# arpan-dhatt/wgpu-n-body

Measured on AMD Instinct MI355X. Metric: body-pair interactions/sec, 64k-body all-pairs, higher is better.
Workload: dtype f32; 1 GPU; 65536-body naive all-pairs step (BASELINE configs[1]), uniform_init seed 2, g=1e-6 e=1e-4 dt=0.016; bodies=65536, parallelism=body-range shard x1, lib=nbody_hip 0.2.0 gfx950 src:823fa9bfdf5b, kernel_variant=auto

## Files before the change

wgpu_n_body_amd/csrc/nb_common.hpp:

```cpp
#pragma once

#include <hip/hip_runtime.h>

#include <cstdarg>
#include <cstddef>
#include <cstdint>
#include <cstdio>
#include <string>

#include "nbody.h"

namespace nb {

void set_error(const char *fmt, ...) __attribute__((format(printf, 1, 2)));

#define NB_HIP_TRY(expr)                                                                       \
    do {                                                                                       \
        hipError_t nb_e_ = (expr);                                                             \
        if (nb_e_ != hipSuccess) {                                                             \
            ::nb::set_error("%s failed: %s (%s:%d)", #expr, hipGetErrorString(nb_e_), __FILE__, \
                            __LINE__);                                                         \
            return NB_ERR_HIP;                                                                 \
        }                                                                                      \
    } while (0)

constexpr uint32_t kWave = 64;
constexpr uint32_t kIB = 2;
constexpr uint32_t kITile = kWave * kIB;
constexpr uint32_t kJTile = 64;
constexpr uint32_t kPadTo = 256;

constexpr int kMaxPeers = 15;
struct PeerDst {
    float4 *p[kMaxPeers];
    uint32_t n;
};

struct PeerWords {
    uint32_t *p[kMaxPeers];
    uint32_t n;
};
hipError_t launch_peer_check_store(const PeerWords &dst, uint32_t slot, uint32_t value, hipStream_t stream);
hipError_t launch_peer_check_read(const uint32_t *words, uint32_t world, uint32_t me, uint32_t tag, uint32_t *bad,
                                  hipStream_t stream);

struct NaiveLaunch {
    const float4 *posm_src;
    float4 *posm_dst;
    float4 *vel;
    float4 *acc;
    uint32_t n;
    uint32_t n_pad;
    uint32_t lo, hi;
    float g, e, dt;
    int variant;
    int jsplit;
    int mass_runs;
    float4 *partial;
    uint32_t partial_stride;
    uint32_t partial_slices;
    int phase;
    PeerDst peers;
};
enum { kPhaseAll = 0, kPhaseLocal = 1, kPhaseRemote = 2 };
struct NaivePlan {
    int variant;
    uint32_t blocks;
    uint32_t jsplit;
    uint32_t js_local, js_remote;
    uint32_t n_tiles, lo_tile, local_tiles;
    bool two_phase;
};
NaivePlan plan_naive(uint32_t n, uint32_t lo, uint32_t hi, int variant, int jsplit, bool two_phase);
hipError_t launch_naive_step(const NaiveLaunch &a, hipStream_t stream);
int naive_variant_count();
const char *naive_variant_name(int v);

hipError_t launch_aos_to_soa(const nb_particle *aos, float4 *posm, float4 *vel, float4 *acc,
                             uint32_t n, uint32_t lo, uint32_t hi, hipStream_t stream);
hipError_t launch_soa_to_aos(const float4 *posm, const float4 *vel, const float4 *acc,
                             nb_particle *aos, uint32_t n, uint32_t lo, uint32_t hi,
                             hipStream_t stream);

}
```

wgpu_n_body_amd/csrc/nb_naive.hip:

```cpp
#include "nb_common.hpp"

#include <type_traits>

namespace nb {
namespace {

typedef float v2f __attribute__((ext_vector_type(2)));
typedef float v4f __attribute__((ext_vector_type(4)));

enum JSource { kLds = 0, kSmem = 1 };

struct TileWindow {
    uint32_t base, count, skip_at, skip_len;
    __device__ __forceinline__ uint32_t tile(uint32_t v) const {
        return base + v + (v >= skip_at ? skip_len : 0u);
    }
};

__device__ __forceinline__ float kick(float v, float a, float dt) {
#pragma clang fp contract(off)
    return v + (a * dt) / 2.0f;
}
__device__ __forceinline__ float drift(float x, float v, float dt) {
#pragma clang fp contract(off)
    return x + v * dt;
}

template <bool MASKED, bool UNIFORM>
__device__ __forceinline__ void pair(float xj, float yj, float zj, float mj, float xi, float yi,
                                     float zi, float e, bool valid, float &ax, float &ay,
                                     float &az) {
    const float dx = xj - xi, dy = yj - yi, dz = zj - zi;
    const float r2 = __builtin_fmaf(dz, dz, __builtin_fmaf(dy, dy, dx * dx));
    const float r = __builtin_amdgcn_sqrtf(r2);
    const float den = __builtin_fmaf(e, r, r2 * r2);
    float w = __builtin_amdgcn_rcpf(den);
    if (!UNIFORM) w *= mj;
    if (MASKED) w = valid ? w : 0.0f;
    ax = __builtin_fmaf(w, dx, ax);
    ay = __builtin_fmaf(w, dy, ay);
    az = __builtin_fmaf(w, dz, az);
}

template <bool MASKED, bool UNIFORM>
__device__ __forceinline__ void pair2(float xj, float yj, float zj, float mj, v2f xi, v2f yi,
                                      v2f zi, float e, bool valid0, bool valid1, v2f &ax,
                                      v2f &ay, v2f &az) {
    const v2f dx = v2f{xj, xj} - xi, dy = v2f{yj, yj} - yi, dz = v2f{zj, zj} - zi;
    const v2f r2 = __builtin_elementwise_fma(dz, dz, __builtin_elementwise_fma(dy, dy, dx * dx));
    v2f r;
    r.x = __builtin_amdgcn_sqrtf(r2.x);
    r.y = __builtin_amdgcn_sqrtf(r2.y);
    const v2f den = __builtin_elementwise_fma(v2f{e, e}, r, r2 * r2);
    v2f rc;
    rc.x = __builtin_amdgcn_rcpf(den.x);
    rc.y = __builtin_amdgcn_rcpf(den.y);
    v2f w = UNIFORM ? rc : v2f{mj, mj} * rc;
    if (MASKED) {
        w.x = valid0 ? w.x : 0.0f;
        w.y = valid1 ? w.y : 0.0f;
    }
    ax = __builtin_elementwise_fma(w, dx, ax);
    ay = __builtin_elementwise_fma(w, dy, ay);
    az = __builtin_elementwise_fma(w, dz, az);
}

template <int IB, int SRC, bool PACKED, bool MASKED, bool UNIFORM, int UNROLL, typename Ptr,
          typename T>
__device__ __forceinline__ void tile_body(Ptr tile, uint32_t j0, uint32_t n, const uint32_t *ii,
                                          const T *xi, const T *yi, const T *zi, float e, T *ax,
                                          T *ay, T *az) {
#pragma unroll UNROLL
    for (uint32_t jj = 0; jj < kJTile; ++jj) {
        float4 pj = tile[jj];
        const uint32_t j = j0 + jj;
        if constexpr (PACKED && UNIFORM && SRC == kLds) {
            v4f q{pj.x, pj.y, pj.z, pj.w};
            asm("" : "+v"(q));
            pj = float4{q.x, q.y, q.z, q.w};
        }
        if constexpr (PACKED) {
#pragma unroll
            for (int k = 0; k < IB / 2; ++k)
                pair2<MASKED, UNIFORM>(pj.x, pj.y, pj.z, pj.w, xi[k], yi[k], zi[k], e,
                                       (j != ii[2 * k]) & (j < n), (j != ii[2 * k + 1]) & (j < n),
                                       ax[k], ay[k], az[k]);
        } else {
#pragma unroll
            for (int k = 0; k < IB; ++k)
                pair<MASKED, UNIFORM>(pj.x, pj.y, pj.z, pj.w, xi[k], yi[k], zi[k], e,
                                      (j != ii[k]) & (j < n), ax[k], ay[k], az[k]);
        }
    }
}

template <typename T>
__device__ __forceinline__ float &elem(T *a, int k);
template <>
__device__ __forceinline__ float &elem<float>(float *a, int k) {
    return a[k];
}
template <>
__device__ __forceinline__ float &elem<v2f>(v2f *a, int k) {
    return reinterpret_cast<float *>(a)[k];
}

template <int IB, int SRC, bool PACKED, int UNROLL, typename Ptr, typename T>
__device__ __forceinline__ void tile_any(bool uniform, bool special, Ptr tile, uint32_t j0,
                                         uint32_t n, const uint32_t *ii, const T *xi, const T *yi,
                                         const T *zi, float e, T *ax, T *ay, T *az) {
    if (uniform) {
        if (special)
            tile_body<IB, SRC, PACKED, true, true, 2>(tile, j0, n, ii, xi, yi, zi, e, ax, ay, az);
        else
            tile_body<IB, SRC, PACKED, false, true, UNROLL>(tile, j0, n, ii, xi, yi, zi, e, ax, ay, az);
    } else {
        if (special)
            tile_body<IB, SRC, PACKED, true, false, 2>(tile, j0, n, ii, xi, yi, zi, e, ax, ay, az);
        else
            tile_body<IB, SRC, PACKED, false, false, UNROLL>(tile, j0, n, ii, xi, yi, zi, e, ax, ay, az);
    }
}

__device__ __forceinline__ bool tile_in_run(float m, uint32_t m_run, uint32_t j0, uint32_t lane,
                                            uint32_t n) {
    const bool differs = (__float_as_uint(m) != m_run) & (j0 + lane < n);
    return __builtin_amdgcn_ballot_w64(differs) == 0;
}

template <int NV, typename T>
__device__ __forceinline__ void scale_sums(uint32_t m_run, T *ax, T *ay, T *az) {
    const float m = __uint_as_float(m_run);
#pragma unroll
    for (int k = 0; k < NV; ++k) {
        ax[k] *= m;
        ay[k] *= m;
        az[k] *= m;
    }
}

template <int IB, int W, int SRC, bool PACKED, int UNROLL>
__global__ __launch_bounds__(64 * W) void naive_step_kernel(
    const float4 *__restrict__ posm_src, float4 *__restrict__ posm_dst, float4 *__restrict__ vel,
    float4 *__restrict__ acc, float4 *__restrict__ partial, uint32_t partial_stride, uint32_t n,
    uint32_t n_pad, uint32_t lo, uint32_t hi, float g, float e, float dt, TileWindow win,
    uint32_t mass_runs) {
    static_assert(!PACKED || IB % 2 == 0, "packed fp32 needs an even number of bodies per lane");
    using T = typename std::conditional<PACKED, v2f, float>::type;
    constexpr int NV = PACKED ? IB / 2 : IB;
    __shared__ float4 s_tile[SRC == kLds ? W * 2 * kJTile : 1];
    __shared__ float s_red[W > 1 ? (W - 1) * IB * 3 * 64 : 1];

    const uint32_t lane = threadIdx.x & 63u;
    const uint32_t wave = __builtin_amdgcn_readfirstlane(threadIdx.x >> 6);
    const uint32_t i0 = lo + blockIdx.x * (64u * IB);
    const uint32_t slot = blockIdx.y * W + wave;
    const uint32_t n_slots = gridDim.y * W;

    uint32_t ii[IB];
    float vhx[IB], vhy[IB], vhz[IB], mi[IB];
    T xi[NV], yi[NV], zi[NV], ax[NV], ay[NV], az[NV];
#pragma unroll
    for (int k = 0; k < IB; ++k) {
        ii[k] = i0 + lane + 64u * k;
        const uint32_t ic = ii[k] < hi ? ii[k] : hi - 1u;
        const float4 p = posm_src[ic];
        const float4 v = vel[ic - lo];
        const float4 a = acc[ic - lo];
        vhx[k] = kick(v.x, a.x, dt);
        vhy[k] = kick(v.y, a.y, dt);
        vhz[k] = kick(v.z, a.z, dt);
        elem<T>(xi, k) = drift(p.x, vhx[k], dt);
        elem<T>(yi, k) = drift(p.y, vhy[k], dt);
        elem<T>(zi, k) = drift(p.z, vhz[k], dt);
        mi[k] = p.w;
        elem<T>(ax, k) = 0.0f;
        elem<T>(ay, k) = 0.0f;
        elem<T>(az, k) = 0.0f;
    }

    const uint32_t n_tiles = (n + kJTile - 1u) / kJTile;
    const uint32_t t_self_lo = i0 / kJTile, t_self_hi = (i0 + 64u * IB - 1u) / kJTile;
    const uint32_t t_ragged = (n % kJTile) ? n_tiles - 1u : ~0u;
    bool in_run = mass_runs != 0u;
    uint32_t m_run;
    if constexpr (SRC == kLds) {
        float4 *my = s_tile + wave * 2 * kJTile;
        uint32_t vt = slot;
        float4 nxt = vt < win.count ? posm_src[win.tile(vt) * kJTile + lane] : float4{0, 0, 0, 0};
        uint32_t buf = 0;
        m_run = __builtin_amdgcn_readfirstlane(__float_as_uint(nxt.w));
        for (; vt < win.count; vt += n_slots) {
            const uint32_t t = win.tile(vt);
            my[buf * kJTile + lane] = nxt;
            if (in_run && !tile_in_run(nxt.w, m_run, t * kJTile, lane, n)) {
                scale_sums<NV>(m_run, ax, ay, az);
                in_run = false;
            }
            __builtin_amdgcn_wave_barrier();
            const uint32_t vn = vt + n_slots;
            if (vn < win.count) nxt = posm_src[win.tile(vn) * kJTile + lane];
            const float4 *tile = my + buf * kJTile;
            const bool special = (t >= t_self_lo && t <= t_self_hi) || t == t_ragged;
            tile_any<IB, SRC, PACKED, UNROLL>(in_run, special, tile, t * kJTile, n, ii, xi, yi, zi, e,
                                              ax, ay, az);
            __builtin_amdgcn_wave_barrier();
            buf ^= 1u;
        }
    } else {
        uint32_t vt = slot;
        float m_nxt = vt < win.count ? posm_src[win.tile(vt) * kJTile + lane].w : 0.0f;
        m_run = __builtin_amdgcn_readfirstlane(__float_as_uint(m_nxt));
        for (; vt < win.count; vt += n_slots) {
            const uint32_t t = win.tile(vt);
            const float4 *tile = posm_src + t * kJTile;
            if (in_run && !tile_in_run(m_nxt, m_run, t * kJTile, lane, n)) {
                scale_sums<NV>(m_run, ax, ay, az);
                in_run = false;
            }
            const uint32_t vn = vt + n_slots;
            if (in_run && vn < win.count) m_nxt = posm_src[win.tile(vn) * kJTile + lane].w;
            const bool special = (t >= t_self_lo && t <= t_self_hi) || t == t_ragged;
            tile_any<IB, SRC, PACKED, UNROLL>(in_run, special, tile, t * kJTile, n, ii, xi, yi, zi, e,
                                              ax, ay, az);
        }
    }
    if (in_run) scale_sums<NV>(m_run, ax, ay, az);

    float sx[IB], sy[IB], sz[IB];
#pragma unroll
    for (int k = 0; k < IB; ++k) {
        sx[k] = elem<T>(ax, k);
        sy[k] = elem<T>(ay, k);
        sz[k] = elem<T>(az, k);
    }
    if constexpr (W > 1) {
        if (wave != 0) {
            float *dst = s_red + (wave - 1u) * (IB * 3 * 64);
#pragma unroll
            for (int k = 0; k < IB; ++k) {
                dst[(k * 3 + 0) * 64 + lane] = sx[k];
                dst[(k * 3 + 1) * 64 + lane] = sy[k];
                dst[(k * 3 + 2) * 64 + lane] = sz[k];
            }
        }
        __syncthreads();
        if (wave != 0) return;
#pragma unroll 1
        for (int w = 1; w < W; ++w) {
            const float *src = s_red + (w - 1) * (IB * 3 * 64);
#pragma unroll
            for (int k = 0; k < IB; ++k) {
                sx[k] += src[(k * 3 + 0) * 64 + lane];
                sy[k] += src[(k * 3 + 1) * 64 + lane];
                sz[k] += src[(k * 3 + 2) * 64 + lane];
            }
        }
    }

    if (partial) {
#pragma unroll
        for (int k = 0; k < IB; ++k)
            if (ii[k] < hi)
                partial[(size_t)blockIdx.y * partial_stride + (ii[k] - lo)] =
                    float4{sx[k], sy[k], sz[k], 0.0f};
        return;
    }

    const float gdt = g * dt;
#pragma unroll
    for (int k = 0; k < IB; ++k) {
        if (ii[k] >= hi) continue;
        const float fx = sx[k] * gdt, fy = sy[k] * gdt, fz = sz[k] * gdt;
        posm_dst[ii[k]] = float4{elem<T>(xi, k), elem<T>(yi, k), elem<T>(zi, k), mi[k]};
        vel[ii[k] - lo] = float4{kick(vhx[k], fx, dt), kick(vhy[k], fy, dt), kick(vhz[k], fz, dt),
                                 0.0f};
        acc[ii[k] - lo] = float4{fx, fy, fz, 0.0f};
    }
}

__global__ __launch_bounds__(256) void naive_finish_kernel(
    const float4 *__restrict__ posm_src, float4 *__restrict__ posm_dst, float4 *__restrict__ vel,
    float4 *__restrict__ acc, const float4 *__restrict__ partial, uint32_t partial_stride,
    uint32_t js, uint32_t lo, uint32_t hi, float g, float dt, PeerDst peers) {
    const uint32_t i = lo + blockIdx.x * blockDim.x + threadIdx.x;
    if (i >= hi) return;
    const float4 p = posm_src[i], v = vel[i - lo], a = acc[i - lo];
    const float vhx = kick(v.x, a.x, dt), vhy = kick(v.y, a.y, dt), vhz = kick(v.z, a.z, dt);
    float sx = 0.0f, sy = 0.0f, sz = 0.0f;
    for (uint32_t s = 0; s < js; ++s) {
        const float4 q = partial[(size_t)s * partial_stride + (i - lo)];
        if (s == 0) {
            sx = q.x; sy = q.y; sz = q.z;
        } else {
            sx += q.x; sy += q.y; sz += q.z;
        }
    }
    const float gdt = g * dt;
    const float fx = sx * gdt, fy = sy * gdt, fz = sz * gdt;
    const float4 pn = float4{drift(p.x, vhx, dt), drift(p.y, vhy, dt), drift(p.z, vhz, dt), p.w};
    posm_dst[i] = pn;
    for (uint32_t k = 0; k < peers.n; ++k) peers.p[k][i] = pn;
    vel[i - lo] = float4{kick(vhx, fx, dt), kick(vhy, fy, dt), kick(vhz, fz, dt), 0.0f};
    acc[i - lo] = float4{fx, fy, fz, 0.0f};
}

__global__ void aos_to_soa_kernel(const nb_particle *__restrict__ aos, float4 *__restrict__ posm,
                                  float4 *__restrict__ vel, float4 *__restrict__ acc, uint32_t n,
                                  uint32_t lo, uint32_t hi) {
    const uint32_t i = blockIdx.x * blockDim.x + threadIdx.x;
    if (i >= n) return;
    const nb_particle p = aos[i];
    posm[i] = float4{p.position[0], p.position[1], p.position[2], p.mass};
    if (i >= lo && i < hi) {
        vel[i - lo] = float4{p.velocity[0], p.velocity[1], p.velocity[2], 0.0f};
        acc[i - lo] = float4{p.acceleration[0], p.acceleration[1], p.acceleration[2], 0.0f};
    }
}

__global__ void soa_to_aos_kernel(const float4 *__restrict__ posm, const float4 *__restrict__ vel,
                                  const float4 *__restrict__ acc, nb_particle *__restrict__ aos,
                                  uint32_t n, uint32_t lo, uint32_t hi) {
    const uint32_t i = blockIdx.x * blockDim.x + threadIdx.x;
    if (i >= n) return;
    const float4 p = posm[i];
    float4 v{0, 0, 0, 0}, a{0, 0, 0, 0};
    if (i >= lo && i < hi) {
        v = vel[i - lo];
        a = acc[i - lo];
    }
    nb_particle o;
    o.position[0] = p.x; o.position[1] = p.y; o.position[2] = p.z;
    o.velocity[0] = v.x; o.velocity[1] = v.y; o.velocity[2] = v.z;
    o.acceleration[0] = a.x; o.acceleration[1] = a.y; o.acceleration[2] = a.z;
    o.mass = p.w;
    aos[i] = o;
}

using KernelFn = void (*)(const float4 *, float4 *, float4 *, float4 *, float4 *, uint32_t,
                          uint32_t, uint32_t, uint32_t, uint32_t, float, float, float, TileWindow,
                          uint32_t);
struct Variant {
    const char *name;
    KernelFn fn;
    int ib, w;
};
#define NB_V(IB, W, SRC, PK, UN) \
    { "ib" #IB "_w" #W "_" #SRC "_pk" #PK "_u" #UN, naive_step_kernel<IB, W, SRC, PK, UN>, IB, W }
const Variant kVariants[] = {
    NB_V(2, 8, kLds, false, 8),
    NB_V(2, 8, kLds, true, 8),
    NB_V(2, 16, kSmem, true, 8),
    NB_V(4, 16, kLds, true, 2),
    NB_V(4, 16, kLds, true, 4),
#ifdef NB_ALL_VARIANTS
    NB_V(2, 8, kSmem, false, 8), NB_V(2, 8, kSmem, true, 8), NB_V(2, 4, kLds, false, 8),
    NB_V(2, 4, kLds, true, 8), NB_V(4, 8, kLds, false, 4), NB_V(4, 8, kLds, true, 4),
    NB_V(4, 4, kLds, true, 4), NB_V(1, 8, kLds, false, 8), NB_V(1, 16, kLds, false, 8),
    NB_V(2, 16, kLds, false, 8), NB_V(2, 16, kLds, true, 8), NB_V(4, 8, kSmem, true, 4),
    NB_V(4, 8, kLds, true, 2), NB_V(4, 16, kSmem, true, 2), NB_V(2, 16, kLds, true, 4),
    NB_V(4, 16, kLds, true, 1), NB_V(8, 16, kLds, true, 1), NB_V(8, 8, kLds, true, 1),
    NB_V(4, 16, kLds, true, 8), NB_V(4, 8, kLds, true, 8), NB_V(2, 16, kLds, true, 16),
    NB_V(4, 16, kSmem, true, 4), NB_V(2, 16, kSmem, true, 16), NB_V(2, 16, kSmem, true, 4),
#endif
};
constexpr int kNumVariants = sizeof(kVariants) / sizeof(kVariants[0]);

constexpr int kAutoVariant = 4;
constexpr uint32_t kTargetBlocks = 256;
constexpr uint32_t kMaxJSplit = 32;

}

int naive_variant_count() { return kNumVariants; }
const char *naive_variant_name(int v) {
    return (v >= 0 && v < kNumVariants) ? kVariants[v].name : "?";
}

static uint32_t pick_jsplit(uint32_t blocks, uint32_t tiles, uint32_t waves, int forced) {
    const uint32_t max_js = tiles / waves ? tiles / waves : 1u;
    uint32_t js = 1;
    if (forced > 0)
        js = (uint32_t)forced;
    else if (blocks && blocks < kTargetBlocks)
        js = (kTargetBlocks + blocks - 1u) / blocks;
    if (js > max_js) js = max_js;
    if (js > kMaxJSplit) js = kMaxJSplit;
    return js ? js : 1u;
}

NaivePlan plan_naive(uint32_t n, uint32_t lo, uint32_t hi, int variant, int jsplit, bool two_phase) {
    NaivePlan p{};
    p.variant = (variant >= 0 && variant < kNumVariants) ? variant : kAutoVariant;
    const Variant &v = kVariants[p.variant];
    const uint32_t itile = 64u * (uint32_t)v.ib;
    const uint32_t n_local = hi > lo ? hi - lo : 0u;
    p.blocks = n_local ? (n_local + itile - 1u) / itile : 0u;
    p.n_tiles = (n + kJTile - 1u) / kJTile;
    p.lo_tile = lo / kJTile;
    p.local_tiles = (n_local + kJTile - 1u) / kJTile;
    p.two_phase = two_phase && n_local > 0 && p.local_tiles < p.n_tiles;
    if (p.two_phase) {
        p.js_local = pick_jsplit(p.blocks, p.local_tiles, (uint32_t)v.w, jsplit);
        p.js_remote = pick_jsplit(p.blocks, p.n_tiles - p.local_tiles, (uint32_t)v.w, jsplit);
        p.jsplit = p.js_local + p.js_remote;
    } else {
        p.jsplit = pick_jsplit(p.blocks, p.n_tiles, (uint32_t)v.w, jsplit);
        p.js_local = 0;
        p.js_remote = p.jsplit;
    }
    return p;
}

hipError_t launch_naive_step(const NaiveLaunch &a, hipStream_t stream) {
    if (a.hi <= a.lo) return hipSuccess;
    const NaivePlan p = plan_naive(a.n, a.lo, a.hi, a.variant, a.jsplit, a.phase != kPhaseAll);
    const Variant &v = kVariants[p.variant];
    const dim3 block(64u * (uint32_t)v.w);
    const uint32_t nl = a.hi - a.lo;
    const uint32_t mr = a.mass_runs ? 1u : 0u;
    if (a.phase == kPhaseAll) {
        if (p.jsplit > 1 && (!a.partial || a.partial_slices < p.jsplit)) return hipErrorInvalidValue;
        const TileWindow all{0u, p.n_tiles, ~0u, 0u};
        hipLaunchKernelGGL(v.fn, dim3(p.blocks, p.jsplit), block, 0, stream, a.posm_src, a.posm_dst,
                           a.vel, a.acc, p.jsplit > 1 ? a.partial : (float4 *)nullptr, a.partial_stride,
                           a.n, a.n_pad, a.lo, a.hi, a.g, a.e, a.dt, all, mr);
        if (p.jsplit > 1)
            hipLaunchKernelGGL(naive_finish_kernel, dim3((nl + 255u) / 256u), dim3(256), 0, stream,
                               a.posm_src, a.posm_dst, a.vel, a.acc, a.partial, a.partial_stride,
                               p.jsplit, a.lo, a.hi, a.g, a.dt, a.peers);
        return hipGetLastError();
    }
    if (!p.two_phase || !a.partial || a.partial_slices < p.jsplit) return hipErrorInvalidValue;
    if (a.phase == kPhaseLocal) {
        const TileWindow own{p.lo_tile, p.local_tiles, ~0u, 0u};
        hipLaunchKernelGGL(v.fn, dim3(p.blocks, p.js_local), block, 0, stream, a.posm_src, a.posm_dst,
                           a.vel, a.acc, a.partial, a.partial_stride, a.n, a.n_pad, a.lo, a.hi, a.g,
                           a.e, a.dt, own, mr);
    } else {
        const TileWindow rest{0u, p.n_tiles - p.local_tiles, p.lo_tile, p.local_tiles};
        hipLaunchKernelGGL(v.fn, dim3(p.blocks, p.js_remote), block, 0, stream, a.posm_src, a.posm_dst,
                           a.vel, a.acc, a.partial + (size_t)p.js_local * a.partial_stride,
                           a.partial_stride, a.n, a.n_pad, a.lo, a.hi, a.g, a.e, a.dt, rest, mr);
        hipLaunchKernelGGL(naive_finish_kernel, dim3((nl + 255u) / 256u), dim3(256), 0, stream,
                           a.posm_src, a.posm_dst, a.vel, a.acc, a.partial, a.partial_stride, p.jsplit,
                           a.lo, a.hi, a.g, a.dt, a.peers);
    }
    return hipGetLastError();
}

hipError_t launch_aos_to_soa(const nb_particle *aos, float4 *posm, float4 *vel, float4 *acc,
                             uint32_t n, uint32_t lo, uint32_t hi, hipStream_t stream) {
    if (n == 0) return hipSuccess;
    hipLaunchKernelGGL(aos_to_soa_kernel, dim3((n + 255u) / 256u), dim3(256), 0, stream, aos, posm,
                       vel, acc, n, lo, hi);
    return hipGetLastError();
}

hipError_t launch_soa_to_aos(const float4 *posm, const float4 *vel, const float4 *acc,
                             nb_particle *aos, uint32_t n, uint32_t lo, uint32_t hi,
                             hipStream_t stream) {
    if (n == 0) return hipSuccess;
    hipLaunchKernelGGL(soa_to_aos_kernel, dim3((n + 255u) / 256u), dim3(256), 0, stream, posm, vel,
                       acc, aos, n, lo, hi);
    return hipGetLastError();
}

__global__ void peer_check_store_kernel(PeerWords dst, uint32_t slot, uint32_t value) {
    const uint32_t q = blockIdx.x * blockDim.x + threadIdx.x;
    if (q < dst.n) dst.p[q][slot] = value;
}
__global__ void peer_check_read_kernel(const uint32_t *__restrict__ words, uint32_t world, uint32_t me, uint32_t tag,
                                       uint32_t *__restrict__ bad) {
    const uint32_t r = blockIdx.x * blockDim.x + threadIdx.x;
    if (r < world && r != me && words[r] != (tag | r)) atomicAdd(bad, 1u);
}

hipError_t launch_peer_check_store(const PeerWords &dst, uint32_t slot, uint32_t value, hipStream_t stream) {
    hipLaunchKernelGGL(peer_check_store_kernel, dim3(1), dim3(64), 0, stream, dst, slot, value);
    return hipGetLastError();
}
hipError_t launch_peer_check_read(const uint32_t *words, uint32_t world, uint32_t me, uint32_t tag, uint32_t *bad,
                                  hipStream_t stream) {
    hipLaunchKernelGGL(peer_check_read_kernel, dim3(1), dim3(64), 0, stream, words, world, me, tag, bad);
    return hipGetLastError();
}

}
```

wgpu_n_body_amd/csrc/nb_sim.hpp:

```cpp
#pragma once

#include <memory>
#include <vector>

#include "nb_common.hpp"

namespace nb {

struct Workspace {
    virtual ~Workspace() = default;
};
enum WorkSlot : int { kWorkDiag = 0, kWorkRender, kWorkRadial, kWorkField, kWorkMap, kWorkFof, kWorkKnn, kWorkSmooth,
                      kWorkBound, kWorkHalo, kWorkHop, kWorkShape, kWorkRadii, kWorkModes, kWorkShell, kWorkPhase, kWorkTidal,
                      kWorkKin, kWorkOrbits, kWorkFof6, kWorkStability, kWorkSlots };

enum ExchangeRegion : int {
    kRegionPositions = 0,
    kRegionVelocities = 1,
    kRegionAccelerations = 2,
    kReplicatedRegions = 3,
    kLetMeta = 0,
    kLetExportCounts = 1,
    kLetExportSegments = 2,
    kLetImportArea = 3,
// ... 117 lines not shown
    uint32_t records;
};
int orbits_check_args(const nb_orbit_params *p, const double *pos, const double *vel, size_t m,
                      const nb_orbit_sample *tracks, OrbitPlan *plan);
int orbits_check_e(const SimBase &sim, const nb_orbit_params *p);
int sim_orbits(SimBase &sim, const nb_orbit_params &params, const OrbitPlan &plan, const double *pos, const double *vel,
               size_t m, nb_orbit_sample *tracks, uint32_t *coincident, nb_orbit_stats *stats);
uint32_t orbit_records(uint32_t steps, uint32_t every);
int orbit_phase(double omega, double dt, uint64_t k, double *c, double *s);
int orbit_sections_check_args(const nb_orbit_params *p, const nb_orbit_section_params *sec, const double *pos,
                              const double *vel, size_t m, const nb_orbit_sample *tracks,
                              const nb_orbit_crossing *crossings, OrbitPlan *plan);
int sim_orbit_sections(SimBase &sim, const nb_orbit_params &params, const nb_orbit_section_params &sec,
                       const OrbitPlan &plan, const double *pos, const double *vel, size_t m, nb_orbit_sample *tracks,
                       uint32_t *coincident, nb_orbit_crossing *crossings, uint32_t *counts,
                       nb_orbit_summary *summaries, nb_orbit_section_stats *stats);
int orbit_summary_merge(const nb_orbit_summary *a, const nb_orbit_summary *b, nb_orbit_summary *out);
int orbit_stability_check_args(const nb_orbit_params *p, const nb_orbit_stability_params *sp, const double *pos,
                               const double *vel, size_t m, const nb_orbit_deviation *dev0,
                               const nb_orbit_sample *tracks, const nb_orbit_deviation *devs, OrbitPlan *plan);
int sim_orbit_stability(SimBase &sim, const nb_orbit_params &params, const nb_orbit_stability_params &sp,
                        const OrbitPlan &plan, const double *pos, const double *vel, size_t m,
                        const nb_orbit_deviation *dev0, nb_orbit_sample *tracks, uint32_t *coincident,
                        nb_orbit_deviation *devs, nb_orbit_growth *growth, nb_orbit_stability_stats *stats);
int orbit_stability_derive(double dt, uint32_t steps, uint32_t every, size_t m, uint32_t deviations,
                           const nb_orbit_deviation *dev0, const nb_orbit_deviation *devs, double *log_growth,
                           double *lyapunov, double *sali, double *gali2);

struct MapPlan {
    double n[3], e1[3], e2[3];
    double dx, dy;
};
int map_check_params(const nb_map_params *p, MapPlan *plan);
int sim_map(SimBase &sim, const nb_map_params &params, const MapPlan &plan, uint32_t *counts, double *planes,
            nb_map_stats *stats);
struct PhasePlan {
    double n[3], e1[3], e2[3];
    bool uses_values;
};
int phase_check_params(const nb_phase_params *p, PhasePlan *plan);
int phase_check_args(const SimBase &sim, const nb_phase_params *p, const PhasePlan &plan);
int sim_phase_map(SimBase &sim, const nb_phase_params &params, const PhasePlan &plan, uint32_t *counts, double *planes,
                  nb_phase_stats *stats);
int phase_quantity(const char *name, uint32_t *id);
const char *phase_quantity_name(uint32_t id);
int fof_check_params(const nb_fof_params *p);
int sim_fof(SimBase &sim, const nb_fof_params &params, uint32_t *labels, uint32_t *group_of, nb_fof_group *groups,
            size_t group_capacity, nb_fof_stats *stats);
int fof6_check_params(const nb_fof6_params *p);
int sim_fof6(SimBase &sim, const nb_fof6_params &params, uint32_t *labels, uint32_t *group_of, nb_fof_group *groups,
             size_t group_capacity, nb_fof_stats *stats);
int halo_check_params(const nb_halo_params *p);
int sim_halo_profiles(SimBase &sim, const nb_halo_params &params, nb_halo_head *heads, nb_radial_bin *bins,
                      nb_halo_stats *stats);

int bound_check_params(const nb_bound_params *p);
int bound_check_e(const SimBase &sim);
int sim_bound(SimBase &sim, const nb_bound_params &params, uint32_t *group_of, uint32_t *bound_of, double *energy,
              nb_bound_group *groups, size_t group_capacity, nb_bound_stats *stats);
int shape_check_params(const nb_shape_params *p);
int shape_check_args(const SimBase &sim, const nb_shape_params *p, const uint32_t *group_of, size_t m,
                     const double *centers, const double *velocities, const double *radius);
int sim_group_shapes(SimBase &sim, const nb_shape_params &params, const uint32_t *group_of, size_t m,
                     const double *centers, const double *velocities, const double *radius, nb_shape_group *rows,
                     uint32_t *selected_of, nb_shape_stats *stats);
void shape_eigen_host(const double t[6], double lambda[3], double axes[9]);
int radii_check_params(const nb_radii_params *p);
int radii_check_args(const SimBase &sim, const nb_radii_params *p, const uint32_t *group_of, size_t m,
                     const double *centers);
int sim_group_radii(SimBase &sim, const nb_radii_params &params, const uint32_t *group_of, size_t m,
                    const double *centers, nb_radii_group *rows, uint32_t *rank_of, double *enclosed_of,
                    nb_radii_stats *stats);
int modes_check_params(const nb_modes_params *p, const nb_modes_head *out, const nb_modes_bin *bins,
                       const double *modes);
int sim_disc_modes(SimBase &sim, const nb_modes_params &params, nb_modes_head *out, nb_modes_bin *bins, double *modes);
int modes_derive(const double *modes, uint32_t nbins, uint32_t mmax, uint32_t m, nb_modes_derived *out);
int shell_check_params(const nb_shell_params *p, const nb_shell_head *out, const nb_shell_bin *bins,
                       const double *coef);
int sim_shell_modes(SimBase &sim, const nb_shell_params &params, nb_shell_head *out, nb_shell_bin *bins, double *coef);
int shell_derive(const nb_shell_head *head, const double *coef, nb_shell_derived *out, double *norm, double *phase,
                 double *speed);
int knn_check_params(const nb_knn_params *p);
int sim_knn(SimBase &sim, const nb_knn_params &params, double *r2, uint32_t *kth, double *mass_in, double *density,
            nb_knn_stats *stats);
int kin_check_params(const nb_kin_params *p);
int sim_local_kinematics(SimBase &sim, const nb_kin_params &params, double *moments, double *grads, double *r2,
                         uint32_t *kth, double *mass_in, double *density, nb_kin_stats *stats);
int kin_derive(const double *moments, const double *grads, const double *r2, const double *density,
               const float *velocities, size_t n, nb_kin_derived *out);
int hop_check_params(const nb_hop_params *p);
int sim_hop(SimBase &sim, const nb_hop_params &params, uint32_t *labels, uint32_t *group_of, double *density,
            nb_fof_group *groups, double *peak_density, size_t group_capacity, nb_hop_boundary *boundaries,
            size_t boundary_capacity, nb_hop_stats *stats);
struct SmoothPlan {
    MapPlan frame;
    std::vector<double> xc, yc;
};
int smooth_check_params(const nb_smooth_params *p, SmoothPlan *plan);
int sim_smooth_map(SimBase &sim, const nb_smooth_params &params, const SmoothPlan &plan, const double *s,
                   uint32_t *counts, double *planes, nb_smooth_stats *stats);
bool axis_frame(const double axis[3], double n[3], double e1[3], double e2[3]);
int radial_lagrangian(const nb_radial_profile *p, const nb_radial_bin *bins, const double *edges,
                      const double *fractions, uint32_t k, double *radii);
int field_rings(const double center[3], const double axis[3], const double *radii, uint32_t k, uint32_t n_phi,
                float *points);
int field_ring_means(const double center[3], const double axis[3], const double *radii, uint32_t k, uint32_t n_phi,
                     const float *points, const nb_field_sample *samples, nb_field_ring *out);
int tidal_ring_means(const double center[3], const double axis[3], const double *radii, uint32_t k, uint32_t n_phi,
                     const float *points, const nb_tidal_sample *samples, const nb_field_ring *rings,
                     nb_tidal_ring *out);
int halo_enclosed(const nb_halo_head *head, const nb_radial_bin *bins, uint32_t nbins, double *out);
int halo_overdensity(const nb_halo_head *head, const nb_radial_bin *bins, const double *edges, uint32_t nbins,
                     double rho, double *r, double *mass);
int hop_regroup(const nb_fof_group *rows, const double *peak_density, size_t m, const nb_hop_boundary *bnd, size_t b,
                const nb_hop_regroup_params *params, uint32_t *merged_of_row, nb_fof_group *out_rows,
                double *out_peak, size_t out_capacity, size_t *out_count);
int map_frame(const double axis[3], double n_hat[3], double e1[3], double e2[3]);
int map_edges(double lo, double hi, uint32_t cells, double *edges);
int smooth_centres(double lo, double hi, uint32_t cells, double *out);

class NaiveSim final : public SimBase {
   public:
    ~NaiveSim() override;
    int init(const nb_particle *host, size_t count) override;
    int encode() override;
    int encode_phase(int phase) override;
    int read_particles(nb_particle *dst, size_t count) override;
    int write_particles(const nb_particle *src, size_t count) override;
    int encode_n_timed(int count, float *ms_total, float *ms_kernel) override;
    int exchange_count() override { return 1; }
    int exchange_region(int index, void **dev_ptr, size_t *off, size_t *len, size_t *total) override;
    int set_tuning(const char *key, int value) override;
    void diag_state(const float4 **posm_out, const float4 **vel_out) const override {
        *posm_out = posm[cur];
        *vel_out = vel;
    }
    void position_buffers(float4 *out[2]) const {
        out[0] = posm[0];
        out[1] = posm[1];
    }
    int set_peers(float4 *const *peer_buf0, float4 *const *peer_buf1, int count);

   private:
    PeerDst peers[2] = {};
    float4 *posm[2] = {nullptr, nullptr};
    bool own_posm = true;
    float4 *vel = nullptr, *acc = nullptr;
    nb_particle *d_aos = nullptr;
    int cur = 0;
    int variant = -1, jsplit = 0;
    int mass_runs = 1;
    float4 *partial = nullptr;
    uint32_t partial_slices = 0;
    int ensure_workspace();
    int launch(int phase);
    bool local_done = false;
    std::vector<hipEvent_t> events;
};

SimBase *make_tree_sim();

nb_add_params add_params_or_default(const nb_add_params *ap);
size_t shard_bodies_per_rank(size_t particle_num, int world);
size_t shard_padded_bodies(size_t particle_num, int world);
int make_sim_impl(std::unique_ptr<SimBase> &out, const nb_sim_params *sp, const nb_add_params *ap,
                  const nb_placement *pl, const nb_particle *particles, size_t count);

}

struct nb_sim {
    std::unique_ptr<nb::SimBase> impl;
};
```

wgpu_n_body_amd/csrc/nb_simbase.cpp:

```cpp
#include <cstdlib>
#include <cstring>
#include <memory>
#include <new>
#include <vector>

#include "nb_common.hpp"
#include "nb_sim.hpp"

namespace nb {

static size_t round_up(size_t x, size_t m) { return (x + m - 1) / m * m; }

size_t shard_bodies_per_rank(size_t particle_num, int world) {
    if (world < 1) world = 1;
    const size_t per = (particle_num + (size_t)world - 1) / (size_t)world;
    return round_up(per ? per : 1, kPadTo);
}

size_t shard_padded_bodies(size_t particle_num, int world) {
    if (world < 1) world = 1;
    return shard_bodies_per_rank(particle_num, world) * (size_t)world;
}

SimBase::~SimBase() {
    for (auto &w : work) w.reset();
    if (own_stream && stream) (void)hipStreamDestroy(stream);
}

int SimBase::setup_common(const nb_sim_params &p, const nb_add_params &ap, const nb_placement *pl) {
    params = p;
    add = ap;
    nb_placement d{};
    d.device_id = 0;
    d.rank = 0;
    d.world = 1;
    place = pl ? *pl : d;
    if (place.world < 1 || place.rank < 0 || place.rank >= place.world) {
        set_error("invalid placement: rank %d of world %d", place.rank, place.world);
        return NB_ERR_INVALID;
    }
    int count = 0;
    if (hipGetDeviceCount(&count) != hipSuccess || count <= 0) {
        set_error("no HIP device is visible (hipGetDeviceCount); there is no CPU fallback");
        return NB_ERR_NO_DEVICE;
    }
    if (place.device_id < 0) place.device_id = 0;
    if (place.device_id >= count) {
        set_error("device_id %d out of range (%d devices)", place.device_id, count);
        return NB_ERR_INVALID;
    }
    NB_HIP_TRY(hipSetDevice(place.device_id));
    if (place.stream) {
        stream = static_cast<hipStream_t>(place.stream);
        own_stream = false;
    } else {
        NB_HIP_TRY(hipStreamCreateWithFlags(&stream, hipStreamNonBlocking));
        own_stream = true;
    }
    n = p.particle_num;
    per_rank = (uint32_t)shard_bodies_per_rank(n, place.world);
    n_pad = (uint32_t)shard_padded_bodies(n, place.world);
    const uint64_t lo64 = (uint64_t)per_rank * (uint64_t)place.rank;
    lo = (uint32_t)(lo64 < n ? lo64 : n);
    const uint64_t hi64 = lo64 + per_rank;
    hi = (uint32_t)(hi64 < n ? hi64 : n);
    return NB_OK;
}

int SimBase::bind_device() const {
    NB_HIP_TRY(hipSetDevice(place.device_id));
    return NB_OK;
}

int SimBase::wait() {
    if (int rc = bind_device()) return rc;
    NB_HIP_TRY(hipStreamSynchronize(stream));
    return NB_OK;
}

NaiveSim::~NaiveSim() {
    (void)hipSetDevice(place.device_id);
    if (own_posm) {
        if (posm[0]) (void)hipFree(posm[0]);
        if (posm[1]) (void)hipFree(posm[1]);
    }
    if (vel) (void)hipFree(vel);
    if (acc) (void)hipFree(acc);
    if (d_aos) (void)hipFree(d_aos);
    if (partial) (void)hipFree(partial);
    for (hipEvent_t e : events) (void)hipEventDestroy(e);
}

int NaiveSim::init(const nb_particle *host, size_t count) {
    if (count != n) {
        set_error("particle count %zu does not match sim_params.particle_num %u", count, n);
        return NB_ERR_INVALID;
    }
    const size_t posm_bytes = sizeof(float4) * (size_t)n_pad;
    if (place.posm[0] || place.posm[1]) {
        if (!place.posm[0] || !place.posm[1] || place.posm[0] == place.posm[1]) {
            set_error("placement.posm needs two distinct device buffers (or none)");
            return NB_ERR_INVALID;
        }
        posm[0] = static_cast<float4 *>(place.posm[0]);
        posm[1] = static_cast<float4 *>(place.posm[1]);
        own_posm = false;
    } else {
        NB_HIP_TRY(hipMalloc(&posm[0], posm_bytes));
        NB_HIP_TRY(hipMalloc(&posm[1], posm_bytes));
        own_posm = true;
    }
    const size_t local_bytes = sizeof(float4) * (size_t)(per_rank ? per_rank : kPadTo);
    NB_HIP_TRY(hipMalloc(&vel, local_bytes));
    NB_HIP_TRY(hipMalloc(&acc, local_bytes));
    NB_HIP_TRY(hipMalloc(&d_aos, sizeof(nb_particle) * (size_t)(n ? n : 1)));
    NB_HIP_TRY(hipMemsetAsync(posm[0], 0, posm_bytes, stream));
    NB_HIP_TRY(hipMemsetAsync(posm[1], 0, posm_bytes, stream));
    NB_HIP_TRY(hipMemsetAsync(vel, 0, local_bytes, stream));
    NB_HIP_TRY(hipMemsetAsync(acc, 0, local_bytes, stream));
    if (const char *v = getenv("NB_NAIVE_VARIANT")) variant = atoi(v);
    if (const char *v = getenv("NB_NAIVE_JSPLIT")) jsplit = atoi(v);
    if (int rc = ensure_workspace()) return rc;
    return write_particles(host, count);
}

int NaiveSim::ensure_workspace() {
    const NaivePlan p1 = plan_naive(n, lo, hi, variant, jsplit, false);
    const NaivePlan p2 = plan_naive(n, lo, hi, variant, jsplit, place.world > 1);
    NaivePlan p = p1;
    if (p2.two_phase && p2.jsplit > p.jsplit) p.jsplit = p2.jsplit;
    if ((p.jsplit > 1 || p2.two_phase) && p.jsplit > partial_slices) {
        if (int rc = bind_device()) return rc;
        NB_HIP_TRY(hipStreamSynchronize(stream));
        if (partial) NB_HIP_TRY(hipFree(partial));
        partial = nullptr;
        partial_slices = 0;
        NB_HIP_TRY(hipMalloc(&partial, sizeof(float4) * (size_t)p.jsplit * (size_t)per_rank));
        partial_slices = p.jsplit;
    }
    return NB_OK;
}

int NaiveSim::write_particles(const nb_particle *host, size_t count) {
    if (count != n) {
        set_error("write_particles: count %zu != particle_num %u", count, n);
        return NB_ERR_INVALID;
    }
    if (int rc = bind_device()) return rc;
    if (n == 0) return NB_OK;
    local_done = false;
    NB_HIP_TRY(hipMemcpyAsync(d_aos, host, sizeof(nb_particle) * (size_t)n, hipMemcpyHostToDevice,
                              stream));
    NB_HIP_TRY(launch_aos_to_soa(d_aos, posm[cur], vel, acc, n, lo, hi, stream));
    NB_HIP_TRY(hipMemcpyAsync(posm[cur ^ 1], posm[cur], sizeof(float4) * (size_t)n_pad,
                              hipMemcpyDeviceToDevice, stream));
    NB_HIP_TRY(hipStreamSynchronize(stream));
    return NB_OK;
}

int NaiveSim::launch(int phase) {
    NaiveLaunch a{};
    a.posm_src = posm[cur];
    a.posm_dst = posm[cur ^ 1];
    a.vel = vel;
    a.acc = acc;
    a.n = n;
    a.n_pad = n_pad;
    a.lo = lo;
    a.hi = hi;
    a.g = params.g;
    a.e = params.e;
    a.dt = params.dt;
    a.variant = variant;
    a.jsplit = jsplit;
    a.mass_runs = mass_runs;
    a.partial = partial;
    a.partial_stride = per_rank;
    a.partial_slices = partial_slices;
    a.phase = phase;
    a.peers = peers[cur ^ 1];
    if (a.peers.n && hi > lo && !(lo == 0 && hi == n)) {
        const NaivePlan p = plan_naive(n, lo, hi, variant, jsplit, phase != kPhaseAll);
        if (phase == kPhaseAll && p.jsplit <= 1) {
            set_error("a NaiveSim with peers steps in two phases (nb_sim_encode_phase)");
            return NB_ERR_INVALID;
        }
    }
    NB_HIP_TRY(launch_naive_step(a, stream));
    return NB_OK;
}

int NaiveSim::encode() {
    if (int rc = bind_device()) return rc;
    if (local_done) return encode_phase(1);
    if (int rc = launch(kPhaseAll)) return rc;
    cur ^= 1;
    step_num += 1;
    return NB_OK;
}

int NaiveSim::encode_phase(int phase) {
    if (int rc = bind_device()) return rc;
    const NaivePlan p = plan_naive(n, lo, hi, variant, jsplit, true);
    if (!p.two_phase) {
        if (phase == 0) return NB_OK;
        if (int rc = launch(kPhaseAll)) return rc;
        cur ^= 1;
        step_num += 1;
        return NB_OK;
    }
    if (phase == 0) {
        if (local_done) {
            set_error("encode_phase(0) called twice for one step");
            return NB_ERR_INVALID;
        }
        if (int rc = launch(kPhaseLocal)) return rc;
        local_done = true;
        return NB_OK;
    }
    if (phase != 1) {
        set_error("encode_phase: phase must be 0 or 1");
        return NB_ERR_INVALID;
    }
    if (!local_done)
        if (int rc = launch(kPhaseLocal)) return rc;
    if (int rc = launch(kPhaseRemote)) return rc;
    local_done = false;
    cur ^= 1;
    step_num += 1;
    return NB_OK;
}

int NaiveSim::encode_n_timed(int count, float *ms_total, float *ms_kernel) {
    if (count <= 0) {
        set_error("encode_n_timed: n must be positive");
        return NB_ERR_INVALID;
    }
    if (int rc = bind_device()) return rc;
    while (events.size() < (size_t)(2 * count + 2)) {
        hipEvent_t e;
        NB_HIP_TRY(hipEventCreate(&e));
        events.push_back(e);
    }
    NB_HIP_TRY(hipEventRecord(events[0], stream));
    for (int k = 0; k < count; ++k) {
        NB_HIP_TRY(hipEventRecord(events[2 + 2 * k], stream));
        if (int rc = encode()) return rc;
        NB_HIP_TRY(hipEventRecord(events[3 + 2 * k], stream));
    }
    NB_HIP_TRY(hipEventRecord(events[1], stream));
    NB_HIP_TRY(hipStreamSynchronize(stream));
    float total = 0.f, ksum = 0.f;
    NB_HIP_TRY(hipEventElapsedTime(&total, events[0], events[1]));
    for (int k = 0; k < count; ++k) {
        float ms = 0.f;
        NB_HIP_TRY(hipEventElapsedTime(&ms, events[2 + 2 * k], events[3 + 2 * k]));
        ksum += ms;
    }
    if (ms_total) *ms_total = total;
    if (ms_kernel) *ms_kernel = ksum / (float)count;
    return NB_OK;
}

int NaiveSim::read_particles(nb_particle *dst, size_t count) {
    if (count > n) {
        set_error("read_particles: asked for %zu of %u particles", count, n);
        return NB_ERR_INVALID;
    }
    if (int rc = bind_device()) return rc;
    if (count == 0) return wait();
    NB_HIP_TRY(launch_soa_to_aos(posm[cur], vel, acc, d_aos, n, lo, hi, stream));
    NB_HIP_TRY(hipMemcpyAsync(dst, d_aos, sizeof(nb_particle) * count, hipMemcpyDeviceToHost,
                              stream));
    NB_HIP_TRY(hipStreamSynchronize(stream));
    return NB_OK;
}

int NaiveSim::exchange_region(int index, void **dev_ptr, size_t *off, size_t *len, size_t *total) {
    if (index != 0) {
        set_error("exchange region %d out of range (NaiveSim has 1)", index);
        return NB_ERR_INVALID;
    }
    if (dev_ptr) *dev_ptr = posm[cur];
    if (off) *off = sizeof(float4) * (size_t)per_rank * (size_t)place.rank;
    if (len) *len = sizeof(float4) * (size_t)per_rank;
    if (total) *total = sizeof(float4) * (size_t)n_pad;
    return NB_OK;
}

int NaiveSim::set_peers(float4 *const *peer_buf0, float4 *const *peer_buf1, int count) {
    if (count < 0 || count > kMaxPeers) {
        set_error("at most %d peers", kMaxPeers);
        return NB_ERR_INVALID;
    }
    for (int k = 0; k < count; ++k) {
        peers[0].p[k] = peer_buf0[k];
        peers[1].p[k] = peer_buf1[k];
    }
    peers[0].n = peers[1].n = (uint32_t)count;
    return NB_OK;
}

int NaiveSim::set_tuning(const char *key, int value) {
    if (strcmp(key, "naive_variant") == 0) {
        if (value >= naive_variant_count()) {
            set_error("naive_variant %d out of range (%d variants)", value, naive_variant_count());
            return NB_ERR_INVALID;
        }
        variant = value;
        return ensure_workspace();
    }
    if (strcmp(key, "naive_jsplit") == 0) {
        if (value < 0 || value > 32) {
            set_error("naive_jsplit %d out of range [0, 32]", value);
            return NB_ERR_INVALID;
        }
        jsplit = value;
        return ensure_workspace();
    }
    if (strcmp(key, "naive_mass_runs") == 0) {
        if (value != 0 && value != 1) {
            set_error("naive_mass_runs %d is neither 0 nor 1", value);
            return NB_ERR_INVALID;
        }
        mass_runs = value;
        return NB_OK;
    }
    set_error("unknown tuning key '%s'", key);
    return NB_ERR_INVALID;
}

nb_add_params add_params_or_default(const nb_add_params *ap) {
    return ap ? *ap : nb_add_params{NB_NAIVE_SIM_PARAMS, 0.f};
}

int make_sim_impl(std::unique_ptr<SimBase> &out, const nb_sim_params *sp, const nb_add_params *ap,
                  const nb_placement *pl, const nb_particle *particles, size_t count) {
    nb_add_params add = add_params_or_default(ap);
    std::unique_ptr<SimBase> impl;
    if (add.kind == NB_NAIVE_SIM_PARAMS) {
        impl.reset(new (std::nothrow) NaiveSim());
    } else if (add.kind == NB_TREE_SIM_PARAMS) {
        impl.reset(make_tree_sim());
        if (!impl) {
            set_error("TreeSim (Barnes-Hut) is not available in this build");
            return NB_ERR_UNSUPPORTED;
        }
        if (!(add.theta > 0.f)) add.theta = NB_DEFAULT_THETA;
        if (pl && (pl->posm[0] || pl->posm[1])) {
            set_error("TreeSim owns its buffers (placement.posm must be NULL)");
            return NB_ERR_INVALID;
        }
    } else {
        set_error("unknown add_params.kind %d", add.kind);
        return NB_ERR_INVALID;
    }
    if (!impl) {
        set_error("out of host memory");
        return NB_ERR_ALLOC;
    }
    if (int rc = impl->setup_common(*sp, add, pl)) return rc;
    if (int rc = impl->init(particles, count)) return rc;
    out = std::move(impl);
    return NB_OK;
}

}
```

Measured before the change: 3669 billion pairs/s.

## Fuse j-split partial reduction into step kernel via last-block ticket

Adds an optional inline finish: each j-slice block writes its partial sums, increments a per-i-block atomic ticket, and the last arriving block sums all slices and performs the kick/drift/store itself, removing the separate finish kernel launch. It also rewrites the intra-block multi-wave reduction so all waves cooperate on the sum, parking velocities in LDS to lower register pressure. The fused path is off by default (inline_finish=0), so only the reduction restructure and the extra kernel arguments affect the default run.

```diff
diff --git a/wgpu_n_body_amd/csrc/nb_common.hpp b/wgpu_n_body_amd/csrc/nb_common.hpp
--- a/wgpu_n_body_amd/csrc/nb_common.hpp
+++ b/wgpu_n_body_amd/csrc/nb_common.hpp
@@ -61,6 +61,9 @@
     uint32_t partial_slices;
     int phase;
     PeerDst peers;
+    int inline_finish;
+    uint32_t *ticket;
+    uint32_t ticket_words;
 };
 enum { kPhaseAll = 0, kPhaseLocal = 1, kPhaseRemote = 2 };
 struct NaivePlan {
diff --git a/wgpu_n_body_amd/csrc/nb_naive.hip b/wgpu_n_body_amd/csrc/nb_naive.hip
--- a/wgpu_n_body_amd/csrc/nb_naive.hip
+++ b/wgpu_n_body_amd/csrc/nb_naive.hip
@@ -139,17 +139,33 @@
     }
 }
 
+typedef uint32_t v4u __attribute__((ext_vector_type(4)));
+constexpr int kFinishLoads = 8;
+constexpr int kAuxSc1 = 16;
+__device__ __forceinline__ __amdgpu_buffer_rsrc_t slice_rsrc(float4 *slice, uint32_t stride) {
+    return __builtin_amdgcn_make_buffer_rsrc((void *)slice, 0, (int)(stride * 16u), 0x00020000);
+}
+__device__ __forceinline__ void store_slice(__amdgpu_buffer_rsrc_t r, uint32_t i, float x, float y, float z) {
+    const v4u v{__float_as_uint(x), __float_as_uint(y), __float_as_uint(z), 0u};
+    __builtin_amdgcn_raw_buffer_store_b128(v, r, (int)(i * 16u), 0, kAuxSc1);
+}
+__device__ __forceinline__ v4u load_slice(__amdgpu_buffer_rsrc_t r, uint32_t i) {
+    return __builtin_amdgcn_raw_buffer_load_b128(r, (int)(i * 16u), 0, kAuxSc1);
+}
+
 template <int IB, int W, int SRC, bool PACKED, int UNROLL>
 __global__ __launch_bounds__(64 * W) void naive_step_kernel(
     const float4 *__restrict__ posm_src, float4 *__restrict__ posm_dst, float4 *__restrict__ vel,
     float4 *__restrict__ acc, float4 *__restrict__ partial, uint32_t partial_stride, uint32_t n,
     uint32_t n_pad, uint32_t lo, uint32_t hi, float g, float e, float dt, TileWindow win,
-    uint32_t mass_runs) {
+    uint32_t mass_runs, uint32_t *__restrict__ ticket, uint32_t slice0, uint32_t slices,
+    PeerDst peers) {
     static_assert(!PACKED || IB % 2 == 0, "packed fp32 needs an even number of bodies per lane");
     using T = typename std::conditional<PACKED, v2f, float>::type;
     constexpr int NV = PACKED ? IB / 2 : IB;
     __shared__ float4 s_tile[SRC == kLds ? W * 2 * kJTile : 1];
-    __shared__ float s_red[W > 1 ? (W - 1) * IB * 3 * 64 : 1];
+    constexpr uint32_t kSums = IB * 3 * 64;
+    __shared__ float s_red[W > 1 ? W * kSums : 1];
 
     const uint32_t lane = threadIdx.x & 63u;
     const uint32_t wave = __builtin_amdgcn_readfirstlane(threadIdx.x >> 6);
@@ -177,6 +193,18 @@
         elem<T>(ax, k) = 0.0f;
         elem<T>(ay, k) = 0.0f;
         elem<T>(az, k) = 0.0f;
+    }
+    uint32_t park = lane;
+    asm("" : "+v"(park));
+    if constexpr (W > 1) {
+        if (wave == 0) {
+#pragma unroll
+            for (int k = 0; k < IB; ++k) {
+                s_red[(k * 3 + 0) * 64 + lane] = vhx[k];
+                s_red[(k * 3 + 1) * 64 + lane] = vhy[k];
+                s_red[(k * 3 + 2) * 64 + lane] = vhz[k];
+            }
+        }
     }
 
     const uint32_t n_tiles = (n + kJTile - 1u) / kJTile;
@@ -235,36 +263,99 @@
         sz[k] = elem<T>(az, k);
     }
     if constexpr (W > 1) {
-        if (wave != 0) {
-            float *dst = s_red + (wave - 1u) * (IB * 3 * 64);
+        if (wave == 0) {
 #pragma unroll
             for (int k = 0; k < IB; ++k) {
-                dst[(k * 3 + 0) * 64 + lane] = sx[k];
-                dst[(k * 3 + 1) * 64 + lane] = sy[k];
-                dst[(k * 3 + 2) * 64 + lane] = sz[k];
+                vhx[k] = s_red[(k * 3 + 0) * 64 + park];
+                vhy[k] = s_red[(k * 3 + 1) * 64 + park];
+                vhz[k] = s_red[(k * 3 + 2) * 64 + park];
             }
+        }
+        float *dst = s_red + wave * kSums;
+#pragma unroll
+        for (int k = 0; k < IB; ++k) {
+            dst[(k * 3 + 0) * 64 + lane] = sx[k];
+            dst[(k * 3 + 1) * 64 + lane] = sy[k];
+            dst[(k * 3 + 2) * 64 + lane] = sz[k];
+        }
+        __syncthreads();
+        for (uint32_t v = threadIdx.x; v < kSums; v += 64u * W) {
+            float s = s_red[v];
+#pragma unroll
+            for (int w = 1; w < W; ++w) s += s_red[w * kSums + v];
+            s_red[v] = s;
         }
         __syncthreads();
         if (wave != 0) return;
-#pragma unroll 1
-        for (int w = 1; w < W; ++w) {
-            const float *src = s_red + (w - 1) * (IB * 3 * 64);
-#pragma unroll
-            for (int k = 0; k < IB; ++k) {
-                sx[k] += src[(k * 3 + 0) * 64 + lane];
-                sy[k] += src[(k * 3 + 1) * 64 + lane];
-                sz[k] += src[(k * 3 + 2) * 64 + lane];
+#pragma unroll
+        for (int k = 0; k < IB; ++k) {
+            sx[k] = s_red[(k * 3 + 0) * 64 + lane];
+            sy[k] = s_red[(k * 3 + 1) * 64 + lane];
+            sz[k] = s_red[(k * 3 + 2) * 64 + lane];
+        }
+    }
+
+    if (partial) {
+        const uint32_t my = slice0 + blockIdx.y;
+        if (!ticket) {
+#pragma unroll
+            for (int k = 0; k < IB; ++k)
+                if (ii[k] < hi)
+                    partial[(size_t)my * partial_stride + (ii[k] - lo)] =
+                        float4{sx[k], sy[k], sz[k], 0.0f};
+            return;
+        }
+        uint32_t il[IB];
+#pragma unroll
+        for (int k = 0; k < IB; ++k) il[k] = (ii[k] < hi ? ii[k] : hi - 1u) - lo;
+        const __amdgpu_buffer_rsrc_t mine = slice_rsrc(partial + (size_t)my * partial_stride, partial_stride);
+#pragma unroll
+        for (int k = 0; k < IB; ++k)
+            if (ii[k] < hi) store_slice(mine, il[k], sx[k], sy[k], sz[k]);
+        asm volatile("s_waitcnt vmcnt(0)" ::: "memory");
+        uint32_t drawn = 0;
+        if (lane == 0)
+            drawn = __hip_atomic_fetch_add(ticket + blockIdx.x, 1u, __ATOMIC_RELAXED, __HIP_MEMORY_SCOPE_AGENT);
+        drawn = __builtin_amdgcn_readfirstlane(drawn);
+        if (drawn != gridDim.y - 1u) return;
+        __builtin_amdgcn_fence(__ATOMIC_ACQUIRE, "agent");
+        if (lane == 0)
+            __hip_atomic_store(ticket + blockIdx.x, 0u, __ATOMIC_RELAXED, __HIP_MEMORY_SCOPE_AGENT);
+        constexpr int CH = IB >= kFinishLoads ? 1 : kFinishLoads / IB;
+        float tx[IB], ty[IB], tz[IB];
+        for (uint32_t s0 = 0; s0 < slices; s0 += CH) {
+            v4u q[CH][IB];
+#pragma unroll
+            for (int c = 0; c < CH; ++c) {
+                const uint32_t s = s0 + c;
+                if (s < slices && s != my) {
+                    const __amdgpu_buffer_rsrc_t r =
+                        slice_rsrc(partial + (size_t)s * partial_stride, partial_stride);
+#pragma unroll
+                    for (int k = 0; k < IB; ++k) q[c][k] = load_slice(r, il[k]);
+                }
             }
-        }
-    }
-
-    if (partial) {
-#pragma unroll
-        for (int k = 0; k < IB; ++k)
-            if (ii[k] < hi)
-                partial[(size_t)blockIdx.y * partial_stride + (ii[k] - lo)] =
-                    float4{sx[k], sy[k], sz[k], 0.0f};
-        return;
+#pragma unroll
+            for (int c = 0; c < CH; ++c) {
+                const uint32_t s = s0 + c;
+                if (s >= slices) break;
+#pragma unroll
+                for (int k = 0; k < IB; ++k) {
+                    const float x = s == my ? sx[k] : __uint_as_float(q[c][k].x);
+                    const float y = s == my ? sy[k] : __uint_as_float(q[c][k].y);
+                    const float z = s == my ? sz[k] : __uint_as_float(q[c][k].z);
+                    tx[k] = s == 0 ? x : tx[k] + x;
+                    ty[k] = s == 0 ? y : ty[k] + y;
+                    tz[k] = s == 0 ? z : tz[k] + z;
+                }
+            }
+        }
+#pragma unroll
+        for (int k = 0; k < IB; ++k) {
+            sx[k] = tx[k];
+            sy[k] = ty[k];
+            sz[k] = tz[k];
+        }
     }
 
     const float gdt = g * dt;
@@ -272,7 +363,9 @@
     for (int k = 0; k < IB; ++k) {
         if (ii[k] >= hi) continue;
         const float fx = sx[k] * gdt, fy = sy[k] * gdt, fz = sz[k] * gdt;
-        posm_dst[ii[k]] = float4{elem<T>(xi, k), elem<T>(yi, k), elem<T>(zi, k), mi[k]};
+        const float4 pn = float4{elem<T>(xi, k), elem<T>(yi, k), elem<T>(zi, k), mi[k]};
+        posm_dst[ii[k]] = pn;
+        for (uint32_t q = 0; q < peers.n; ++q) peers.p[q][ii[k]] = pn;
         vel[ii[k] - lo] = float4{kick(vhx[k], fx, dt), kick(vhy[k], fy, dt), kick(vhz[k], fz, dt),
                                  0.0f};
         acc[ii[k] - lo] = float4{fx, fy, fz, 0.0f};
@@ -339,7 +432,7 @@
 
 using KernelFn = void (*)(const float4 *, float4 *, float4 *, float4 *, float4 *, uint32_t,
                           uint32_t, uint32_t, uint32_t, uint32_t, float, float, float, TileWindow,
-                          uint32_t);
+                          uint32_t, uint32_t *, uint32_t, uint32_t, PeerDst);
 struct Variant {
     const char *name;
     KernelFn fn;
@@ -419,33 +512,31 @@
     const dim3 block(64u * (uint32_t)v.w);
     const uint32_t nl = a.hi - a.lo;
     const uint32_t mr = a.mass_runs ? 1u : 0u;
-    if (a.phase == kPhaseAll) {
-        if (p.jsplit > 1 && (!a.partial || a.partial_slices < p.jsplit)) return hipErrorInvalidValue;
-        const TileWindow all{0u, p.n_tiles, ~0u, 0u};
-        hipLaunchKernelGGL(v.fn, dim3(p.blocks, p.jsplit), block, 0, stream, a.posm_src, a.posm_dst,
-                           a.vel, a.acc, p.jsplit > 1 ? a.partial : (float4 *)nullptr, a.partial_stride,
-                           a.n, a.n_pad, a.lo, a.hi, a.g, a.e, a.dt, all, mr);
-        if (p.jsplit > 1)
-            hipLaunchKernelGGL(naive_finish_kernel, dim3((nl + 255u) / 256u), dim3(256), 0, stream,
-                               a.posm_src, a.posm_dst, a.vel, a.acc, a.partial, a.partial_stride,
-                               p.jsplit, a.lo, a.hi, a.g, a.dt, a.peers);
-        return hipGetLastError();
-    }
-    if (!p.two_phase || !a.partial || a.partial_slices < p.jsplit) return hipErrorInvalidValue;
+    const bool split = a.phase != kPhaseAll || p.jsplit > 1;
+    if (a.phase != kPhaseAll && !p.two_phase) return hipErrorInvalidValue;
+    if (split && (!a.partial || a.partial_slices < p.jsplit || a.partial_stride < nl)) return hipErrorInvalidValue;
+    const bool finishes = split && a.phase != kPhaseLocal;
+    const bool fused = finishes && a.inline_finish;
+    if (fused && (!a.ticket || a.ticket_words < p.blocks)) return hipErrorInvalidValue;
+    const PeerDst none{};
+    TileWindow win{0u, p.n_tiles, ~0u, 0u};
+    uint32_t slice0 = 0, launched = p.jsplit;
     if (a.phase == kPhaseLocal) {
-        const TileWindow own{p.lo_tile, p.local_tiles, ~0u, 0u};
-        hipLaunchKernelGGL(v.fn, dim3(p.blocks, p.js_local), block, 0, stream, a.posm_src, a.posm_dst,
-                           a.vel, a.acc, a.partial, a.partial_stride, a.n, a.n_pad, a.lo, a.hi, a.g,
-                           a.e, a.dt, own, mr);
-    } else {
-        const TileWindow rest{0u, p.n_tiles - p.local_tiles, p.lo_tile, p.local_tiles};
-        hipLaunchKernelGGL(v.fn, dim3(p.blocks, p.js_remote), block, 0, stream, a.posm_src, a.posm_dst,
-                           a.vel, a.acc, a.partial + (size_t)p.js_local * a.partial_stride,
-                           a.partial_stride, a.n, a.n_pad, a.lo, a.hi, a.g, a.e, a.dt, rest, mr);
-        hipLaunchKernelGGL(naive_finish_kernel, dim3((nl + 255u) / 256u), dim3(256), 0, stream,
-                           a.posm_src, a.posm_dst, a.vel, a.acc, a.partial, a.partial_stride, p.jsplit,
-                           a.lo, a.hi, a.g, a.dt, a.peers);
-    }
+        win = TileWindow{p.lo_tile, p.local_tiles, ~0u, 0u};
+        launched = p.js_local;
+    } else if (a.phase == kPhaseRemote) {
+        win = TileWindow{0u, p.n_tiles - p.local_tiles, p.lo_tile, p.local_tiles};
+        slice0 = p.js_local;
+        launched = p.js_remote;
+    }
+    hipLaunchKernelGGL(v.fn, dim3(p.blocks, launched), block, 0, stream, a.posm_src, a.posm_dst, a.vel, a.acc,
+                       split ? a.partial : (float4 *)nullptr, a.partial_stride, a.n, a.n_pad, a.lo, a.hi, a.g, a.e,
+                       a.dt, win, mr, fused ? a.ticket : (uint32_t *)nullptr, slice0, p.jsplit,
+                       fused ? a.peers : none);
+    if (finishes && !fused)
+        hipLaunchKernelGGL(naive_finish_kernel, dim3((nl + 255u) / 256u), dim3(256), 0, stream, a.posm_src,
+                           a.posm_dst, a.vel, a.acc, a.partial, a.partial_stride, p.jsplit, a.lo, a.hi, a.g, a.dt,
+                           a.peers);
     return hipGetLastError();
 }
 
diff --git a/wgpu_n_body_amd/csrc/nb_sim.hpp b/wgpu_n_body_amd/csrc/nb_sim.hpp
--- a/wgpu_n_body_amd/csrc/nb_sim.hpp
+++ b/wgpu_n_body_amd/csrc/nb_sim.hpp
@@ -293,6 +293,9 @@
     int mass_runs = 1;
     float4 *partial = nullptr;
     uint32_t partial_slices = 0;
+    int inline_finish = 0;
+    uint32_t *ticket = nullptr;
+    uint32_t ticket_words = 0;
     int ensure_workspace();
     int launch(int phase);
     bool local_done = false;
diff --git a/wgpu_n_body_amd/csrc/nb_simbase.cpp b/wgpu_n_body_amd/csrc/nb_simbase.cpp
--- a/wgpu_n_body_amd/csrc/nb_simbase.cpp
+++ b/wgpu_n_body_amd/csrc/nb_simbase.cpp
@@ -88,6 +88,7 @@
     if (acc) (void)hipFree(acc);
     if (d_aos) (void)hipFree(d_aos);
     if (partial) (void)hipFree(partial);
+    if (ticket) (void)hipFree(ticket);
     for (hipEvent_t e : events) (void)hipEventDestroy(e);
 }
 
@@ -120,6 +121,7 @@
     NB_HIP_TRY(hipMemsetAsync(acc, 0, local_bytes, stream));
     if (const char *v = getenv("NB_NAIVE_VARIANT")) variant = atoi(v);
     if (const char *v = getenv("NB_NAIVE_JSPLIT")) jsplit = atoi(v);
+    if (const char *v = getenv("NB_NAIVE_INLINE_FINISH")) inline_finish = atoi(v) != 0;
     if (int rc = ensure_workspace()) return rc;
     return write_particles(host, count);
 }
@@ -137,6 +139,19 @@
         partial_slices = 0;
         NB_HIP_TRY(hipMalloc(&partial, sizeof(float4) * (size_t)p.jsplit * (size_t)per_rank));
         partial_slices = p.jsplit;
+    }
+    if (p.jsplit > 1 || p2.two_phase) {
+        if (int rc = bind_device()) return rc;
+        if (p.blocks > ticket_words) {
+            NB_HIP_TRY(hipStreamSynchronize(stream));
+            if (ticket) NB_HIP_TRY(hipFree(ticket));
+            ticket = nullptr;
+            ticket_words = 0;
+            const uint32_t words = (uint32_t)round_up(p.blocks, 4);
+            NB_HIP_TRY(hipMalloc(&ticket, sizeof(uint32_t) * (size_t)words));
+            ticket_words = words;
+        }
+        if (ticket) NB_HIP_TRY(hipMemsetAsync(ticket, 0, sizeof(uint32_t) * (size_t)ticket_words, stream));
     }
     return NB_OK;
 }
@@ -179,6 +194,9 @@
     a.partial_slices = partial_slices;
     a.phase = phase;
     a.peers = peers[cur ^ 1];
+    a.inline_finish = inline_finish;
+    a.ticket = ticket;
+    a.ticket_words = ticket_words;
     if (a.peers.n && hi > lo && !(lo == 0 && hi == n)) {
         const NaivePlan p = plan_naive(n, lo, hi, variant, jsplit, phase != kPhaseAll);
         if (phase == kPhaseAll && p.jsplit <= 1) {
@@ -324,6 +342,14 @@
             return NB_ERR_INVALID;
         }
         mass_runs = value;
+        return NB_OK;
+    }
+    if (strcmp(key, "naive_inline_finish") == 0) {
+        if (value != 0 && value != 1) {
+            set_error("naive_inline_finish %d is neither 0 nor 1", value);
+            return NB_ERR_INVALID;
+        }
+        inline_finish = value;
         return NB_OK;
     }
     set_error("unknown tuning key '%s'", key);
```

Measured after the change: 3672 billion pairs/s, median of 3. No clear change (+0.1%).
